# 6dwavenminer/Unsynchronized_Stereo_Vision_Proj325

Measured on NVIDIA B200. Metric: frame-pairs/sec, higher is better.
Workload: dtype u8

## Files before the change

### unsynchronized_stereo_vision_proj325_b200/csrc/usv_capi.cu

```cuda
#include <cuda_runtime.h>

#include <atomic>
#include <cmath>
#include <cstdarg>
#include <cstdio>
#include <algorithm>
#include <cstring>
#include <initializer_list>
#include <memory>
#include <new>
#include <vector>

#include "usv_common.cuh"

namespace usv {
cudaError_t launch_direct(const DevJob& J, int n_pairs, cudaStream_t st);
bool direct_supported(const DevJob& J);
size_t dense_scratch_bytes_per_pair(const DevJob& J);
cudaError_t launch_dense(const DevJob& J, int n_pairs, void* d_scratch, size_t scratch_bytes, cudaStream_t st, const char** kernel_name,
                         int* n_launches);
size_t corr_scratch_bytes_per_pair(const DevJob& J);
cudaError_t launch_dense_corr(const DevJob& J, int n_pairs, void* d_scratch, size_t scratch_bytes, cudaStream_t st, const char** kernel_name,
                              int* n_launches);
cudaError_t launch_contour_descriptors(const int* pts, const int* off, int n, double* desc, cudaStream_t st);
cudaError_t launch_contour_costs(const double* dl, int nl, const double* dr, int nr, double* cost, cudaStream_t st);
size_t resolve_workspace_bytes(long long n);
cudaError_t launch_resolve(const usv_match* d_in, long long n, int skip_unmatched, usv_match* d_out, long long cap, long long* d_n_out,
                           void* d_ws, size_t ws_bytes, cudaStream_t st, int* n_launches);
size_t id_matcher_workspace_bytes(long long n_cur);
bool resolve_rows_supported(int nx, int nxc);
struct ResolveRowsSrc {
  const uint16_t* disparity_u16;
  const uint16_t* raw_cost_u16;
  const uint32_t* raw_cost;
  const uint32_t* right_index;
  const usv_match* matches;
};
cudaError_t launch_resolve_rows(const ResolveRowsSrc& S, bool integer_values, int nx, int ny, int sx, int nxc, long long n_templates,
                                int camera_side, int n_pairs, uint16_t* d_out, cudaStream_t st);
cudaError_t launch_id_matcher(const usv_match* d_cur, long long n_cur, const usv_match* d_old, long long n_old, int* d_out3,
                              long long cap, long long* d_n_out, void* d_ws, size_t ws_bytes, cudaStream_t st);
size_t preprocess_scratch_bytes(int width, int height, int n_frames);
cudaError_t launch_preprocess(int device, const uint8_t* d_src, uint8_t* d_dst, const short* d_map1, const uint16_t* d_map2, int n_frames,
                              int width, int height, int src_stride, int dst_stride, long long src_frame_stride,
                              long long dst_frame_stride, int flavour, int lighting, void* d_scratch, cudaStream_t st, int* n_launches);
cudaError_t run_issue_probe(int which, int sms, double target_ms, double* lane_inst_per_s, uint32_t* d_scratch, cudaStream_t st);
cudaError_t launch_disparity_to_distance(const int* d_disp, long long n, int kind, double* d_out, cudaStream_t st);
cudaError_t launch_build_distance_lut(double* d_lut, int n, int kind, cudaStream_t st);
cudaError_t launch_match_list_distance(const usv_match* d_list, const long long* d_n, long long cap, int nx, int sx, int nxc, int camera_side,
                                       int kind, const double* lut, int lut_n, double* d_out, cudaStream_t st);
cudaError_t launch_moving_object_distance(int camera_side, long long t_this, const float* this_xy, int n_this, const float* other_xy,
                                          int n_other, const float* old_xy, int n_old, const float* older_xy, int n_older,
                                          const int* idx3, int n_idx, long long t_other, long long t_old, long long t_older,
                                          double* out, cudaStream_t st);
cudaError_t launch_coordinate_position(int camera_side, const double* dist, const float* xy, long long n, double* xyz, cudaStream_t st);
cudaError_t launch_subpixel_refine(const DevJob& J, int n_pairs, const uint32_t* d_right_index, int* d_x16, double* d_dist,
                                   cudaStream_t st);
}

namespace usv { int g_sm_count = 148; }

using usv::DevJob;

template <bool kPinned>
struct Buf {
  void* p = nullptr;
  size_t cap = 0;
  Buf() = default;
  Buf(const Buf&) = delete;
  Buf& operator=(const Buf&) = delete;
  Buf(Buf&& o) noexcept : p(o.p), cap(o.cap) { o.p = nullptr; o.cap = 0; }
  ~Buf() { release(); }
  cudaError_t release() {
    const cudaError_t e = !p ? cudaSuccess : kPinned ? cudaFreeHost(p) : cudaFree(p);
    p = nullptr;
    cap = 0;
    return e;
  }
  cudaError_t alloc(size_t bytes, unsigned host_flags = cudaHostAllocDefault) {
    const cudaError_t e = kPinned ? cudaHostAlloc(&p, bytes, host_flags) : cudaMalloc(&p, bytes);
    if (e == cudaSuccess) cap = bytes;
    else p = nullptr;
    return e;
  }
};
using DevBuf = Buf<false>;
using PinnedBuf = Buf<true>;

static const int kNumOut = 9;
static const size_t kOutElem[kNumOut] = {sizeof(usv_match), 4, 4, 8, 8, 4, 2, 2, 2};

struct usv_ctx {
  int device = 0;
  cudaStream_t stream = nullptr;
  char err[512] = {0};
  std::atomic<long long> launches{0};
  const char* last_kernel = "none";
  DevBuf lut[3];
  int lut_n[3] = {0, 0, 0};
  std::vector<DevBuf> retired;
  PinnedBuf status;
  int* d_status = nullptr;
  int corr_kernel = USV_CORR_KERNEL_AUTO;
  std::atomic<int> open_streams{0};
  PinnedBuf pin[3];
  DevBuf in_l, in_r, tx, ty, rows_u32, rows_f64, out[kNumOut], misc[8], resolve_ws, pre_ws, corr_ws, win_ws;
  DevBuf sub_ri, sub_x16, sub_dist;
  ~usv_ctx() { if (stream) cudaStreamDestroy(stream); }
};

static int fail(usv_ctx* c, int code, const char* fmt, ...) {
  if (c) {
    va_list ap;
    va_start(ap, fmt);
    vsnprintf(c->err, sizeof(c->err), fmt, ap);
    va_end(ap);
  }
  return code;
}
#define CU(call)                                                                                         \
  do {                                                                                                   \
    cudaError_t e_ = (call);                                                                             \
    if (e_ != cudaSuccess) return fail(ctx, USV_ERR_CUDA, "%s: %s (%s:%d)", #call, cudaGetErrorString(e_), __FILE__, __LINE__); \
  } while (0)

template <bool kPinned>
static int grow(usv_ctx* ctx, Buf<kPinned>& b, size_t bytes) {
  if (bytes <= b.cap) return USV_OK;
  CU(b.release());
  const size_t want = bytes + bytes / 4 + (kPinned ? 4096 : 256);
  const cudaError_t e = b.alloc(want);
  if (e != cudaSuccess)
    return fail(ctx, USV_ERR_NOMEM, "%s(%zu): %s", kPinned ? "cudaHostAlloc" : "cudaMalloc", want, cudaGetErrorString(e));
  return USV_OK;
}

static const size_t kPairScratchCap = (size_t)3 << 29;

static int grow_pair_scratch(usv_ctx* ctx, DevBuf& ws, size_t per_pair, int32_t n_pairs) {
  size_t want = per_pair * (size_t)n_pairs;
  if (want > kPairScratchCap) want = std::max(per_pair, kPairScratchCap / per_pair * per_pair);
  return grow(ctx, ws, want);
}

struct ArrayOrScratch {
  void** arr;
  size_t bytes;
};
static int or_scratch(usv_ctx* ctx, DevBuf& ws, std::initializer_list<ArrayOrScratch> arrs) {
  size_t total = 0;
  for (const ArrayOrScratch& a : arrs) total += *a.arr ? 0 : a.bytes;
  const int rc = grow(ctx, ws, total);
  if (rc) return rc;
  uint8_t* q = (uint8_t*)ws.p;
  for (const ArrayOrScratch& a : arrs)
    if (!*a.arr) { *a.arr = q; q += a.bytes; }
  return USV_OK;
}

static usv_frame_desc device_frame_desc(const usv_frame_desc* f) {
  usv_frame_desc d = *f;
  d.row_stride = (f->width * f->channels + 127) & ~127;
  d.frame_stride = (int64_t)d.row_stride * f->height;
  return d;
}

static int copy_frames(usv_ctx* ctx, uint8_t* dst, const usv_frame_desc& df, const uint8_t* src, const usv_frame_desc* hf, int32_t n,
                       cudaStream_t st) {
  const int row_bytes = hf->width * hf->channels;
  const bool packed = n == 1 || hf->frame_stride == (int64_t)hf->row_stride * hf->height;
  if (packed && hf->row_stride == df.row_stride) {
    CU(cudaMemcpyAsync(dst, src, (size_t)df.frame_stride * n, cudaMemcpyHostToDevice, st));
  } else if (packed) {
    CU(cudaMemcpy2DAsync(dst, df.row_stride, src, hf->row_stride, row_bytes, (size_t)hf->height * n, cudaMemcpyHostToDevice, st));
  } else {
    for (int i = 0; i < n; ++i)
      CU(cudaMemcpy2DAsync(dst + (size_t)i * df.frame_stride, df.row_stride, src + (size_t)i * hf->frame_stride, hf->row_stride,
                           row_bytes, hf->height, cudaMemcpyHostToDevice, st));
  }
  return USV_OK;
}

static void** out_slot(usv_outputs* o, int i) {
  switch (i) {
    case 0: return (void**)&o->matches;
    case 1: return (void**)&o->right_index;
    case 2: return (void**)&o->raw_cost;
    case 3: return (void**)&o->score;
    case 4: return (void**)&o->distance;
    case 5: return (void**)&o->distance_f32;
    case 6: return (void**)&o->disparity_u16;
    case 7: return (void**)&o->raw_cost_u16;
    default: return (void**)&o->resolved_disparity_u16;
  }
}

static int check_common(usv_ctx* ctx, const usv_frame_desc* f, const usv_search_params* p, int32_t n_pairs) {
  if (!ctx) return USV_ERR_INVALID_ARG;
  if (!f || !p) return fail(ctx, USV_ERR_INVALID_ARG, "null frame/params");
  if (n_pairs < 0 || n_pairs > 65535) return fail(ctx, USV_ERR_INVALID_ARG, "n_pairs %d out of [0, 65535]", n_pairs);
  if (f->width <= 0 || f->height <= 0 || f->channels < 1 || f->channels > 4)
    return fail(ctx, USV_ERR_INVALID_ARG, "bad frame %dx%dx%d", f->width, f->height, f->channels);
  if (f->row_stride < f->width * f->channels) return fail(ctx, USV_ERR_INVALID_ARG, "row_stride %d < width*channels", f->row_stride);
  if (n_pairs > 1 && f->frame_stride < (int64_t)f->row_stride * f->height)
    return fail(ctx, USV_ERR_INVALID_ARG, "frame_stride smaller than one frame");
  if (p->tmpl_w <= 0 || p->tmpl_h <= 0 || p->tmpl_w > f->width || p->tmpl_h > f->height)
    return fail(ctx, USV_ERR_INVALID_ARG, "template %dx%d does not fit frame %dx%d", p->tmpl_w, p->tmpl_h, f->width, f->height);
  if ((int64_t)p->tmpl_w * p->tmpl_h * f->channels > 32768)
    return fail(ctx, USV_ERR_UNSUPPORTED, "template of %lld bytes exceeds 32768 (u32 cost accumulators)",
                (long long)p->tmpl_w * p->tmpl_h * f->channels);
  if (p->tmpl_w * f->channels > 1024) return fail(ctx, USV_ERR_UNSUPPORTED, "template row wider than 1024 bytes");
  if (p->stride_x <= 0 || p->stride_y <= 0) return fail(ctx, USV_ERR_INVALID_ARG, "stride must be positive");
  if (p->search_min > p->search_max) return fail(ctx, USV_ERR_INVALID_ARG, "search_min > search_max");
  if (p->search_min < -(1 << 24) || p->search_max > (1 << 24)) return fail(ctx, USV_ERR_INVALID_ARG, "search range beyond +-2^24");
  if (p->cost_kind < USV_COST_SAD || p->cost_kind > USV_COST_ZNCC) return fail(ctx, USV_ERR_INVALID_ARG, "unknown cost_kind %d", p->cost_kind);
  if (p->distance_kind < USV_DIST_NONE || p->distance_kind > USV_DIST_POWERLAW)
    return fail(ctx, USV_ERR_INVALID_ARG, "unknown distance_kind %d", p->distance_kind);
  if (p->camera_side != USV_LEFT_CAM && p->camera_side != USV_RIGHT_CAM) return fail(ctx, USV_ERR_INVALID_ARG, "camera_side must be 0 or 1");
  return USV_OK;
}

static int check_cost_u16(usv_ctx* ctx, const usv_frame_desc* f, const usv_search_params* p) {
  if (p->cost_kind != USV_COST_SAD || 255ll * p->tmpl_w * p->tmpl_h * f->channels >= 0xFFFFll)
    return fail(ctx, USV_ERR_UNSUPPORTED, "raw_cost_u16 needs SAD with 255*tmpl_w*tmpl_h*channels < 65535");
  return USV_OK;
}

static int check_direct(usv_ctx* ctx, const DevJob& J) {
  if (!usv::direct_supported(J))
    return fail(ctx, USV_ERR_UNSUPPORTED, "template %dx%dx%d: no kernel serves this shape (direct form: shared memory)", J.tw, J.th,
                J.channels);
  return USV_OK;
}

static int check_dev_status(usv_ctx* ctx) {
  volatile int* h_status = (volatile int*)ctx->status.p;
  if (h_status && *h_status != 0) {
    const int s = *h_status;
    *h_status = 0;
    return fail(ctx, USV_ERR_CUDA, "device status %d: a kernel abandoned a wait (results of the affected call are invalid)", s);
  }
  return USV_OK;
}

static void fill_job(usv_ctx* ctx, DevJob& J, const uint8_t* l, const uint8_t* r, const usv_frame_desc* f, const usv_search_params* p,
                     const usv_outputs* o) {
  memset(&J, 0, sizeof(J));
  J.status = ctx->d_status;
  J.corr_kernel = ctx->corr_kernel;
  J.left = l; J.right = r;
  J.frame_stride = f->frame_stride;
  J.width = f->width; J.height = f->height; J.channels = f->channels; J.row_stride = f->row_stride;
  J.tw = p->tmpl_w; J.th = p->tmpl_h; J.dmin = p->search_min; J.dmax = p->search_max;
  J.sx = p->stride_x; J.sy = p->stride_y;
  J.cost_kind = p->cost_kind; J.camera_side = p->camera_side; J.distance_kind = p->distance_kind;
  J.nxc = f->width - p->tmpl_w + 1; J.nyc = f->height - p->tmpl_h + 1;
  J.nx = (J.nxc - 1) / p->stride_x + 1; J.ny = (J.nyc - 1) / p->stride_y + 1;
  J.row_bytes = p->tmpl_w * f->channels;
  J.n_elems = p->tmpl_w * p->tmpl_h * f->channels;
  J.accept_threshold = p->accept_threshold;
  J.n_templates = J.nx * J.ny;
  if (o) J.out = *o;
}

static int ensure_lut(usv_ctx* ctx, int kind, int width, cudaStream_t st, const double** lut) {
  *lut = nullptr;
  if (kind == USV_DIST_NONE) return USV_OK;
  if (ctx->lut_n[kind] < width) {
    if (ctx->lut[kind].p) { ctx->retired.push_back(std::move(ctx->lut[kind])); ctx->lut_n[kind] = 0; }
    int n = width < 4096 ? 4096 : width;
    CU(ctx->lut[kind].alloc(sizeof(double) * n));
    CU(usv::launch_build_distance_lut((double*)ctx->lut[kind].p, n, kind, st));
    CU(cudaStreamSynchronize(st));
    ctx->launches++;
    ctx->lut_n[kind] = n;
  }
  *lut = (const double*)ctx->lut[kind].p;
  return USV_OK;
}

static bool aligned16(const void* p) { return (reinterpret_cast<uintptr_t>(p) & 15) == 0; }

extern "C" int usv_abi_version(void) { return USV_ABI_VERSION; }

extern "C" int usv_create(int device, usv_ctx** out) {
  if (!out) return USV_ERR_INVALID_ARG;
  *out = nullptr;
  int n = 0;
  cudaError_t e = cudaGetDeviceCount(&n);
  if (e != cudaSuccess || n <= 0) return USV_ERR_NO_DEVICE;
  if (device < 0 || device >= n) return USV_ERR_INVALID_ARG;
  if (cudaSetDevice(device) != cudaSuccess) return USV_ERR_CUDA;
  cudaDeviceProp prop;
  if (cudaGetDeviceProperties(&prop, device) != cudaSuccess) return USV_ERR_CUDA;
  if (prop.major != 10 || prop.minor != 0) return USV_ERR_NO_DEVICE;
  usv_ctx* c = new (std::nothrow) usv_ctx();
  if (!c) return USV_ERR_NOMEM;
  c->device = device;
  usv::g_sm_count = prop.multiProcessorCount;
  if (cudaStreamCreateWithFlags(&c->stream, cudaStreamNonBlocking) != cudaSuccess ||
      c->status.alloc(sizeof(int), cudaHostAllocMapped) != cudaSuccess ||
      cudaHostGetDevicePointer((void**)&c->d_status, c->status.p, 0) != cudaSuccess) {
    delete c;
    return USV_ERR_CUDA;
  }
  *(int*)c->status.p = 0;
  *out = c;
  return USV_OK;
}

extern "C" int usv_destroy(usv_ctx* ctx) {
  if (!ctx) return USV_ERR_INVALID_ARG;
  if (ctx->open_streams.load() > 0)
    return fail(ctx, USV_ERR_INVALID_ARG, "%d usv_stream(s) of this context are still open: destroy them first", ctx->open_streams.load());
  cudaSetDevice(ctx->device);
  cudaStreamSynchronize(ctx->stream);
  delete ctx;
  return USV_OK;
}

extern "C" const char* usv_last_error(const usv_ctx* ctx) { return ctx ? ctx->err : "null context"; }
extern "C" int64_t usv_launch_count(const usv_ctx* ctx) { return ctx ? (int64_t)ctx->launches.load() : -1; }
extern "C" const char* usv_last_kernel(const usv_ctx* ctx) { return ctx ? ctx->last_kernel : "none"; }
extern "C" int usv_set_option(usv_ctx* ctx, int32_t key, int64_t value) {
  if (!ctx) return USV_ERR_INVALID_ARG;
  if (key == USV_OPT_CORR_KERNEL) {
    if (value < USV_CORR_KERNEL_AUTO || value > USV_CORR_KERNEL_TCGEN05) return fail(ctx, USV_ERR_INVALID_ARG, "USV_OPT_CORR_KERNEL: value %lld", (long long)value);
    ctx->corr_kernel = (int)value;
    return USV_OK;
  }
  return fail(ctx, USV_ERR_INVALID_ARG, "unknown option %d", key);
}
extern "C" int usv_device_status(usv_ctx* ctx) { return ctx ? check_dev_status(ctx) : USV_ERR_INVALID_ARG; }

extern "C" int usv_grid_dims(const usv_frame_desc* f, const usv_search_params* p, int32_t* nx, int32_t* ny, int64_t* cand_evals) {
  if (!f || !p) return USV_ERR_INVALID_ARG;
  int nxc = f->width - p->tmpl_w + 1, nyc = f->height - p->tmpl_h + 1;
  if (nxc <= 0 || nyc <= 0 || p->stride_x <= 0 || p->stride_y <= 0) return USV_ERR_INVALID_ARG;
  int gx = (nxc - 1) / p->stride_x + 1, gy = (nyc - 1) / p->stride_y + 1;
  int64_t per_row = 0;
  for (int ix = 0; ix < gx; ++ix) {
    int lo, hi;
    usv::cand_range(ix * p->stride_x, nxc, p->camera_side, p->search_min, p->search_max, &lo, &hi);
    if (hi >= lo) per_row += hi - lo + 1;
  }
  if (nx) *nx = gx;
  if (ny) *ny = gy;
  if (cand_evals) *cand_evals = per_row * gy;
  return USV_OK;
}

static int resolve_device(usv_ctx* ctx, const usv_match* d_in, int64_t n, int32_t skip_unmatched, usv_match* d_out, int64_t cap,
                          int64_t* d_n_out, cudaStream_t st);

static int dispatch_match(usv_ctx* ctx, const DevJob& J, int32_t n_pairs, bool sparse, cudaStream_t st, DevBuf* corr_ws) {
  int rc;
  if (!sparse) {
    const char* name = nullptr;
    int nl = 0;
    DevBuf& ws = corr_ws ? *corr_ws : ctx->corr_ws;
    const bool sad_sweep = J.cost_kind == USV_COST_SAD && J.corr_kernel != USV_CORR_KERNEL_ALU;
    if ((rc = grow_pair_scratch(ctx, ws, sad_sweep ? usv::dense_scratch_bytes_per_pair(J) : 0, n_pairs))) return rc;
    cudaError_t e = (J.cost_kind == USV_COST_SAD && J.channels == 3 && J.corr_kernel == USV_CORR_KERNEL_ALU)
                        ? cudaErrorNotSupported
                        : usv::launch_dense(J, n_pairs, ws.p, ws.cap, st, &name, &nl);
    if (e == cudaSuccess) {
      ctx->launches += nl;
      ctx->last_kernel = name;
      return USV_OK;
    }
    if (e != cudaErrorNotSupported) return fail(ctx, USV_ERR_CUDA, "dense launch: %s", cudaGetErrorString(e));
    (void)cudaGetLastError();
    if ((rc = grow_pair_scratch(ctx, ws, usv::corr_scratch_bytes_per_pair(J), n_pairs))) return rc;
    e = usv::launch_dense_corr(J, n_pairs, ws.p, ws.cap, st, &name, &nl);
    if (e == cudaSuccess) {
      ctx->launches += nl;
      ctx->last_kernel = name;
      return USV_OK;
    }
    if (e != cudaErrorNotSupported) return fail(ctx, USV_ERR_CUDA, "dense correlation launch: %s", cudaGetErrorString(e));
    (void)cudaGetLastError();
  }
  if ((rc = check_direct(ctx, J))) return rc;
  cudaError_t e = usv::launch_direct(J, n_pairs, st);
  if (e != cudaSuccess) return fail(ctx, USV_ERR_CUDA, "direct launch: %s", cudaGetErrorString(e));
  ctx->launches++;
  ctx->last_kernel = "block_cost_argmin_direct";
  return USV_OK;
}

enum WinnerSrc { kWinDisparity, kWinRightIndex, kWinMatches };

static WinnerSrc winner_src(const usv_search_params* p, const usv_outputs& o) {
  if (p->cost_kind > USV_COST_SSD) return kWinMatches;
  const bool disp_ok = p->search_min >= 0;
  if (disp_ok && o.disparity_u16 && (o.raw_cost_u16 || o.raw_cost)) return kWinDisparity;
  if (o.right_index && o.raw_cost) return kWinRightIndex;
  return disp_ok ? kWinDisparity : kWinRightIndex;
}

static int match_device(usv_ctx* ctx, const uint8_t* d_left, const uint8_t* d_right, const usv_frame_desc* f, int32_t n_pairs,
                        const usv_search_params* p, const usv_outputs* d_out, const int32_t* d_tx, const int32_t* d_ty,
                        int32_t n_templates, uint32_t* d_cost_rows, double* d_score_rows, int32_t row_cap, cudaStream_t st, DevBuf* corr_ws = nullptr,
                        DevBuf* win_ws = nullptr) {
  int rc = check_common(ctx, f, p, n_pairs);
  if (rc) return rc;
  if (!d_left || !d_right || !d_out) return fail(ctx, USV_ERR_INVALID_ARG, "null device pointer");
  if (!aligned16(d_left) || !aligned16(d_right) || (f->row_stride & 15) || (f->frame_stride & 15))
    return fail(ctx, USV_ERR_INVALID_ARG, "device frames need 16-byte aligned base, row_stride and frame_stride");
  if (d_out->raw_cost_u16 && (rc = check_cost_u16(ctx, f, p))) return rc;
  if (n_pairs == 0) return USV_OK;
  CU(cudaSetDevice(ctx->device));
  DevJob J;
  fill_job(ctx, J, d_left, d_right, f, p, d_out);
  const bool sparse = d_tx != nullptr;
  if (sparse) {
    if (!d_ty || n_templates < 0) return fail(ctx, USV_ERR_INVALID_ARG, "bad template list");
    if (n_templates == 0) return USV_OK;
    J.tx = d_tx; J.ty = d_ty; J.n_templates = n_templates;
    J.cost_rows = d_cost_rows; J.score_rows = d_score_rows; J.row_cap = row_cap;
    if ((d_cost_rows || d_score_rows) && row_cap <= 0) return fail(ctx, USV_ERR_INVALID_ARG, "row_cap must be positive");
  }
  if (J.out.distance || J.out.distance_f32) {
    rc = ensure_lut(ctx, p->distance_kind, f->width, st, &J.dist_lut);
    if (rc) return rc;
  }
  const bool want_resolved = d_out->resolved_disparity_u16 != nullptr;
  const WinnerSrc src = winner_src(p, J.out);
  if (want_resolved) {
    if (sparse) return fail(ctx, USV_ERR_UNSUPPORTED, "resolved_disparity_u16 is an output of the dense sweep");
    if (!usv::resolve_rows_supported(J.nx, J.nxc)) return fail(ctx, USV_ERR_UNSUPPORTED, "resolved_disparity_u16: rows wider than 2048 windows");
    const size_t n_res = (size_t)J.n_templates * n_pairs;
    DevBuf& ws = win_ws ? *win_ws : ctx->win_ws;
    usv_outputs& o = J.out;
    if (src == kWinDisparity)
      rc = or_scratch(ctx, ws, {{o.raw_cost_u16 ? (void**)&o.raw_cost_u16 : (void**)&o.raw_cost, 4 * n_res},
                                {(void**)&o.disparity_u16, 2 * n_res}});
    else if (src == kWinRightIndex)
      rc = or_scratch(ctx, ws, {{(void**)&o.raw_cost, 4 * n_res}, {(void**)&o.right_index, 4 * n_res}});
    else
      rc = or_scratch(ctx, ws, {{(void**)&o.matches, sizeof(usv_match) * n_res}});
    if (rc) return rc;
  }
  if ((rc = dispatch_match(ctx, J, n_pairs, sparse, st, corr_ws))) return rc;
  if (want_resolved) {
    usv::ResolveRowsSrc S;
    memset(&S, 0, sizeof(S));
    if (src == kWinDisparity) {
      S.disparity_u16 = J.out.disparity_u16; S.raw_cost_u16 = J.out.raw_cost_u16; S.raw_cost = J.out.raw_cost;
    } else if (src == kWinRightIndex) {
      S.right_index = J.out.right_index; S.raw_cost = J.out.raw_cost;
    } else {
      S.matches = J.out.matches;
    }
    cudaError_t e = usv::launch_resolve_rows(S, src != kWinMatches, J.nx, J.ny, J.sx, J.nxc, J.n_templates, J.camera_side, n_pairs,
                                             d_out->resolved_disparity_u16, st);
    if (e != cudaSuccess) return fail(ctx, USV_ERR_CUDA, "resolve rows launch: %s", cudaGetErrorString(e));
    ctx->launches++;
  }
  return USV_OK;
}

extern "C" int usv_match_dense_device(usv_ctx* ctx, const uint8_t* d_left, const uint8_t* d_right, const usv_frame_desc* frame,
                                      int32_t n_pairs, const usv_search_params* params, const usv_outputs* d_out, void* cuda_stream) {
  if (!ctx) return USV_ERR_INVALID_ARG;
  return match_device(ctx, d_left, d_right, frame, n_pairs, params, d_out, nullptr, nullptr, 0, nullptr, nullptr, 0,
                      (cudaStream_t)cuda_stream);
}

extern "C" int usv_match_templates_device(usv_ctx* ctx, const uint8_t* d_left, const uint8_t* d_right, const usv_frame_desc* frame,
                                          int32_t n_pairs, const int32_t* d_tx, const int32_t* d_ty, int32_t n_templates,
                                          const usv_search_params* params, const usv_outputs* d_out, uint32_t* d_cost_rows,
                                          double* d_score_rows, int32_t row_cap, void* cuda_stream) {
  if (!ctx) return USV_ERR_INVALID_ARG;
  if (!d_tx) return fail(ctx, USV_ERR_INVALID_ARG, "null template list");
  return match_device(ctx, d_left, d_right, frame, n_pairs, params, d_out, d_tx, d_ty, n_templates, d_cost_rows, d_score_rows,
                      row_cap, (cudaStream_t)cuda_stream);
}

static int check_subpixel(usv_ctx* ctx, const usv_frame_desc* f, const void* x16, const void* dist) {
  if (!x16 && !dist) return fail(ctx, USV_ERR_INVALID_ARG, "sub-pixel refinement: both output pointers are NULL");
  if (f->width > (1 << 26)) return fail(ctx, USV_ERR_UNSUPPORTED, "sub-pixel refinement: frame wider than 2^26 pixels");
  return USV_OK;
}

static int refine_device(usv_ctx* ctx, const uint8_t* d_left, const uint8_t* d_right, const usv_frame_desc* f, int32_t n_pairs,
                         const usv_search_params* p, const uint32_t* d_ri, int32_t* d_x16, double* d_dist, cudaStream_t st) {
  int rc = check_common(ctx, f, p, n_pairs);
  if (rc || (rc = check_subpixel(ctx, f, d_x16, d_dist))) return rc;
  if (!d_left || !d_right || !d_ri) return fail(ctx, USV_ERR_INVALID_ARG, "null device pointer");
  if (!aligned16(d_left) || !aligned16(d_right) || (f->row_stride & 15) || (f->frame_stride & 15))
    return fail(ctx, USV_ERR_INVALID_ARG, "device frames need 16-byte aligned base, row_stride and frame_stride");
  if (n_pairs == 0) return USV_OK;
  CU(cudaSetDevice(ctx->device));
  DevJob J;
  fill_job(ctx, J, d_left, d_right, f, p, nullptr);
  cudaError_t e = usv::launch_subpixel_refine(J, n_pairs, d_ri, d_x16, d_dist, st);
  if (e != cudaSuccess) return fail(ctx, USV_ERR_CUDA, "sub-pixel launch: %s", cudaGetErrorString(e));
  ctx->launches++;
  return USV_OK;
}

extern "C" int usv_refine_subpixel_device(usv_ctx* ctx, const uint8_t* d_left, const uint8_t* d_right, const usv_frame_desc* frame,
                                          int32_t n_pairs, const usv_search_params* params, const uint32_t* d_right_index,
                                          int32_t* d_disparity_x16, double* d_distance, void* cuda_stream) {
  if (!ctx) return USV_ERR_INVALID_ARG;
  return refine_device(ctx, d_left, d_right, frame, n_pairs, params, d_right_index, d_disparity_x16, d_distance,
                       (cudaStream_t)cuda_stream);
}

struct SubpixelOut {
  int32_t* disparity_x16;
  double* distance;
};

static int match_host(usv_ctx* ctx, const uint8_t* h_left, const uint8_t* h_right, const usv_frame_desc* f, int32_t n_pairs,
                      const usv_search_params* p, const usv_outputs* h_out, const int32_t* h_tx, const int32_t* h_ty,
                      int32_t n_templates, uint32_t* h_cost_rows, double* h_score_rows, int32_t row_cap,
                      const SubpixelOut* sub = nullptr) {
  int rc = check_common(ctx, f, p, n_pairs);
  if (rc) return rc;
  if (!h_left || !h_right || !h_out) return fail(ctx, USV_ERR_INVALID_ARG, "null host pointer");
  if (sub && (rc = check_subpixel(ctx, f, sub->disparity_x16, sub->distance))) return rc;
  if (n_pairs == 0) return USV_OK;
  CU(cudaSetDevice(ctx->device));
  cudaStream_t st = ctx->stream;
  const bool sparse = h_tx != nullptr;
  int64_t n_win;
  if (sparse) {
    if (!h_ty || n_templates < 0) return fail(ctx, USV_ERR_INVALID_ARG, "bad template list");
    const int nxc = f->width - p->tmpl_w + 1, nyc = f->height - p->tmpl_h + 1;
    for (int i = 0; i < n_templates; ++i)
      if (h_tx[i] < 0 || h_tx[i] >= nxc || h_ty[i] < 0 || h_ty[i] >= nyc)
        return fail(ctx, USV_ERR_INVALID_ARG, "template %d at (%d,%d) outside the frame", i, h_tx[i], h_ty[i]);
    n_win = n_templates;
    if (n_templates == 0) return USV_OK;
    DevJob J;
    fill_job(ctx, J, nullptr, nullptr, f, p, nullptr);
    if ((rc = check_direct(ctx, J))) return rc;
  } else {
    int32_t nx, ny;
    if (usv_grid_dims(f, p, &nx, &ny, nullptr)) return fail(ctx, USV_ERR_INVALID_ARG, "bad geometry");
    n_win = (int64_t)nx * ny;
  }
  const int64_t n_res = n_win * n_pairs;
  const usv_frame_desc df = device_frame_desc(f);
  const size_t fbytes = (size_t)df.frame_stride * n_pairs;
  if ((rc = grow(ctx, ctx->in_l, fbytes)) || (rc = copy_frames(ctx, (uint8_t*)ctx->in_l.p, df, h_left, f, n_pairs, st))) return rc;
  if ((rc = grow(ctx, ctx->in_r, fbytes)) || (rc = copy_frames(ctx, (uint8_t*)ctx->in_r.p, df, h_right, f, n_pairs, st))) return rc;
  usv_outputs d_out;
  memset(&d_out, 0, sizeof(d_out));
  usv_outputs ho = *h_out;
  for (int i = 0; i < kNumOut; ++i) {
    if (*out_slot(&ho, i)) {
      if ((rc = grow(ctx, ctx->out[i], kOutElem[i] * n_res))) return rc;
      *out_slot(&d_out, i) = ctx->out[i].p;
    }
  }
  int32_t *d_tx = nullptr, *d_ty = nullptr;
  uint32_t* d_rows = nullptr;
  double* d_srows = nullptr;
  if (sparse) {
    if ((rc = grow(ctx, ctx->tx, sizeof(int32_t) * n_templates))) return rc;
    if ((rc = grow(ctx, ctx->ty, sizeof(int32_t) * n_templates))) return rc;
    d_tx = (int32_t*)ctx->tx.p; d_ty = (int32_t*)ctx->ty.p;
    CU(cudaMemcpyAsync(d_tx, h_tx, sizeof(int32_t) * n_templates, cudaMemcpyHostToDevice, st));
    CU(cudaMemcpyAsync(d_ty, h_ty, sizeof(int32_t) * n_templates, cudaMemcpyHostToDevice, st));
    if (h_cost_rows) {
      if ((rc = grow(ctx, ctx->rows_u32, sizeof(uint32_t) * n_res * row_cap))) return rc;
      d_rows = (uint32_t*)ctx->rows_u32.p;
      CU(cudaMemcpyAsync(d_rows, h_cost_rows, sizeof(uint32_t) * n_res * row_cap, cudaMemcpyHostToDevice, st));
    }
    if (h_score_rows) {
      if ((rc = grow(ctx, ctx->rows_f64, sizeof(double) * n_res * row_cap))) return rc;
      d_srows = (double*)ctx->rows_f64.p;
      CU(cudaMemcpyAsync(d_srows, h_score_rows, sizeof(double) * n_res * row_cap, cudaMemcpyHostToDevice, st));
    }
  }
  if (sub && (rc = or_scratch(ctx, ctx->sub_ri, {{(void**)&d_out.right_index, 4 * (size_t)n_res}}))) return rc;
  rc = match_device(ctx, (const uint8_t*)ctx->in_l.p, (const uint8_t*)ctx->in_r.p, &df, n_pairs, p, &d_out, d_tx, d_ty, n_templates,
                    d_rows, d_srows, row_cap, st);
  if (rc) return rc;
  if (sub) {
    int32_t* d_x16 = nullptr;
    double* d_dist = nullptr;
    if (sub->disparity_x16) {
      if ((rc = grow(ctx, ctx->sub_x16, 4 * n_res))) return rc;
      d_x16 = (int32_t*)ctx->sub_x16.p;
    }
    if (sub->distance) {
      if ((rc = grow(ctx, ctx->sub_dist, 8 * n_res))) return rc;
      d_dist = (double*)ctx->sub_dist.p;
    }
    if ((rc = refine_device(ctx, (const uint8_t*)ctx->in_l.p, (const uint8_t*)ctx->in_r.p, &df, n_pairs, p, d_out.right_index, d_x16,
                            d_dist, st)))
      return rc;
    if (d_x16) CU(cudaMemcpyAsync(sub->disparity_x16, d_x16, 4 * n_res, cudaMemcpyDeviceToHost, st));
    if (d_dist) CU(cudaMemcpyAsync(sub->distance, d_dist, 8 * n_res, cudaMemcpyDeviceToHost, st));
  }
  for (int i = 0; i < kNumOut; ++i)
    if (*out_slot(&ho, i)) CU(cudaMemcpyAsync(*out_slot(&ho, i), ctx->out[i].p, kOutElem[i] * n_res, cudaMemcpyDeviceToHost, st));
  if (d_rows) CU(cudaMemcpyAsync(h_cost_rows, d_rows, sizeof(uint32_t) * n_res * row_cap, cudaMemcpyDeviceToHost, st));
  if (d_srows) CU(cudaMemcpyAsync(h_score_rows, d_srows, sizeof(double) * n_res * row_cap, cudaMemcpyDeviceToHost, st));
  CU(cudaStreamSynchronize(st));
  return check_dev_status(ctx);
}

extern "C" int usv_match_dense_host(usv_ctx* ctx, const uint8_t* h_left, const uint8_t* h_right, const usv_frame_desc* frame,
                                    int32_t n_pairs, const usv_search_params* params, const usv_outputs* h_out) {
  if (!ctx) return USV_ERR_INVALID_ARG;
  return match_host(ctx, h_left, h_right, frame, n_pairs, params, h_out, nullptr, nullptr, 0, nullptr, nullptr, 0);
}

extern "C" int usv_match_templates_host(usv_ctx* ctx, const uint8_t* h_left, const uint8_t* h_right, const usv_frame_desc* frame,
                                        int32_t n_pairs, const int32_t* h_tx, const int32_t* h_ty, int32_t n_templates,
                                        const usv_search_params* params, const usv_outputs* h_out, uint32_t* h_cost_rows,
                                        double* h_score_rows, int32_t row_cap) {
  if (!ctx) return USV_ERR_INVALID_ARG;
  if (!h_tx) return fail(ctx, USV_ERR_INVALID_ARG, "null template list");
  return match_host(ctx, h_left, h_right, frame, n_pairs, params, h_out, h_tx, h_ty, n_templates, h_cost_rows, h_score_rows, row_cap);
}

extern "C" int usv_match_dense_subpixel_host(usv_ctx* ctx, const uint8_t* h_left, const uint8_t* h_right, const usv_frame_desc* frame,
                                             int32_t n_pairs, const usv_search_params* params, const usv_outputs* h_out,
                                             int32_t* h_disparity_x16, double* h_distance) {
  if (!ctx) return USV_ERR_INVALID_ARG;
  usv_outputs none;
  memset(&none, 0, sizeof(none));
  const SubpixelOut sub = {h_disparity_x16, h_distance};
  return match_host(ctx, h_left, h_right, frame, n_pairs, params, h_out ? h_out : &none, nullptr, nullptr, 0, nullptr, nullptr, 0, &sub);
}

static int up(usv_ctx* ctx, DevBuf& b, const void* h, size_t bytes) {
  int rc = grow(ctx, b, bytes ? bytes : 16);
  if (rc) return rc;
  if (bytes) CU(cudaMemcpyAsync(b.p, h, bytes, cudaMemcpyHostToDevice, ctx->stream));
  return USV_OK;
}

static int resolve_device(usv_ctx* ctx, const usv_match* d_in, int64_t n, int32_t skip_unmatched, usv_match* d_out, int64_t cap,
                          int64_t* d_n_out, cudaStream_t st) {
  if (n < 0 || cap < 0 || n >= 0x7fffffffll) return fail(ctx, USV_ERR_INVALID_ARG, "match list length %lld out of range", (long long)n);
  if (!d_n_out || (n > 0 && (!d_in || (cap > 0 && !d_out)))) return fail(ctx, USV_ERR_INVALID_ARG, "null pointer");
  CU(cudaSetDevice(ctx->device));
  const size_t ws = n ? usv::resolve_workspace_bytes(n) : 0;
  int rc = grow(ctx, ctx->resolve_ws, ws ? ws : 16);
  if (rc) return rc;
  int nl = 0;
  cudaError_t e = usv::launch_resolve(d_in, n, skip_unmatched, d_out, cap, (long long*)d_n_out, ctx->resolve_ws.p, ws, st, &nl);
  if (e != cudaSuccess) return fail(ctx, USV_ERR_CUDA, "resolve launch: %s", cudaGetErrorString(e));
  ctx->launches += nl;
  if (nl) ctx->last_kernel = "resolve_next_smaller_kernel";
  return USV_OK;
}

extern "C" int usv_resolve_match_list_device(usv_ctx* ctx, const usv_match* d_in, int64_t n, int32_t skip_unmatched, usv_match* d_out,
                                             int64_t cap, int64_t* d_n_out, void* cuda_stream) {
  if (!ctx) return USV_ERR_INVALID_ARG;
  return resolve_device(ctx, d_in, n, skip_unmatched, d_out, cap, d_n_out, (cudaStream_t)cuda_stream);
}

extern "C" int usv_resolve_match_list(usv_ctx* ctx, const usv_match* h_in, int64_t n, int32_t skip_unmatched, usv_match* h_out,
                                      int64_t cap, int64_t* n_out) {
  if (!ctx) return USV_ERR_INVALID_ARG;
  if (n < 0 || cap < 0 || !n_out || (n > 0 && !h_in) || (cap > 0 && !h_out)) return fail(ctx, USV_ERR_INVALID_ARG, "bad arguments");
  *n_out = 0;
  if (n == 0) return USV_OK;
  CU(cudaSetDevice(ctx->device));
  int rc;
  const int64_t room = cap < n ? cap : n;
  if ((rc = up(ctx, ctx->misc[0], h_in, sizeof(usv_match) * (size_t)n))) return rc;
  if ((rc = grow(ctx, ctx->misc[1], sizeof(usv_match) * (size_t)(room ? room : 1)))) return rc;
  if ((rc = grow(ctx, ctx->misc[2], sizeof(int64_t)))) return rc;
  if ((rc = resolve_device(ctx, (const usv_match*)ctx->misc[0].p, n, skip_unmatched, (usv_match*)ctx->misc[1].p, room,
                           (int64_t*)ctx->misc[2].p, ctx->stream)))
    return rc;
  int64_t total = 0;
  CU(cudaMemcpyAsync(&total, ctx->misc[2].p, sizeof(int64_t), cudaMemcpyDeviceToHost, ctx->stream));
  CU(cudaStreamSynchronize(ctx->stream));
  const int64_t m = total < room ? total : room;
  if (m > 0) CU(cudaMemcpy(h_out, ctx->misc[1].p, sizeof(usv_match) * (size_t)m, cudaMemcpyDeviceToHost));
  *n_out = total;
  return USV_OK;
}

extern "C" int usv_block_search_host(usv_ctx* ctx, const uint8_t* h_left, const uint8_t* h_right, const usv_frame_desc* f,
                                     const usv_search_params* p, usv_match* h_matches, double* h_distance, int64_t cap, int64_t* n_out) {
  if (!ctx) return USV_ERR_INVALID_ARG;
  int rc = check_common(ctx, f, p, 1);
  if (rc) return rc;
  if (!h_left || !h_right || !n_out || cap < 0 || (cap > 0 && !h_matches)) return fail(ctx, USV_ERR_INVALID_ARG, "bad arguments");
  *n_out = 0;
  int32_t nx, ny;
  if (usv_grid_dims(f, p, &nx, &ny, nullptr)) return fail(ctx, USV_ERR_INVALID_ARG, "bad geometry");
  const int64_t n_win = (int64_t)nx * ny;
  CU(cudaSetDevice(ctx->device));
  cudaStream_t st = ctx->stream;
  const usv_frame_desc df = device_frame_desc(f);
  const int row_bytes = f->width * f->channels, pitch = df.row_stride;
  const size_t fbytes = (size_t)df.frame_stride;
  if ((rc = grow(ctx, ctx->pin[0], 2 * fbytes))) return rc;
  uint8_t* stage = (uint8_t*)ctx->pin[0].p;
  for (int k = 0; k < 2; ++k) {
    const uint8_t* src = k ? h_right : h_left;
    uint8_t* dst = stage + k * fbytes;
    if (f->row_stride == pitch) memcpy(dst, src, fbytes);
    else for (int y = 0; y < f->height; ++y) memcpy(dst + (size_t)y * pitch, src + (size_t)y * f->row_stride, row_bytes);
  }
  if ((rc = grow(ctx, ctx->in_l, fbytes)) || (rc = grow(ctx, ctx->in_r, fbytes))) return rc;
  CU(cudaMemcpyAsync(ctx->in_l.p, stage, fbytes, cudaMemcpyHostToDevice, st));
  CU(cudaMemcpyAsync(ctx->in_r.p, stage + fbytes, fbytes, cudaMemcpyHostToDevice, st));
  if ((rc = grow(ctx, ctx->out[0], sizeof(usv_match) * n_win))) return rc;
  usv_outputs d_out;
  memset(&d_out, 0, sizeof(d_out));
  d_out.matches = (usv_match*)ctx->out[0].p;
  if ((rc = match_device(ctx, (const uint8_t*)ctx->in_l.p, (const uint8_t*)ctx->in_r.p, &df, 1, p, &d_out, nullptr, nullptr, 0, nullptr,
                         nullptr, 0, st)))
    return rc;
  const char* match_kernel = ctx->last_kernel;
  if ((rc = grow(ctx, ctx->misc[1], sizeof(usv_match) * n_win)) || (rc = grow(ctx, ctx->misc[2], sizeof(int64_t)))) return rc;
  if ((rc = resolve_device(ctx, d_out.matches, n_win, 1, (usv_match*)ctx->misc[1].p, n_win, (int64_t*)ctx->misc[2].p, st))) return rc;
  const bool want_dist = h_distance != nullptr && p->distance_kind != USV_DIST_NONE;
  if (want_dist) {
    const double* lut = nullptr;
    if ((rc = ensure_lut(ctx, p->distance_kind, f->width, st, &lut))) return rc;
    if ((rc = grow(ctx, ctx->misc[3], sizeof(double) * n_win))) return rc;
    CU(usv::launch_match_list_distance((const usv_match*)ctx->misc[1].p, (const long long*)ctx->misc[2].p, n_win, nx, p->stride_x,
                                       f->width - p->tmpl_w + 1, p->camera_side, p->distance_kind, lut, ctx->lut_n[p->distance_kind],
                                       (double*)ctx->misc[3].p, st));
    ctx->launches++;
  }
  ctx->last_kernel = match_kernel;
  if ((rc = grow(ctx, ctx->pin[1], sizeof(usv_match) * n_win + 64)) || (rc = grow(ctx, ctx->pin[2], sizeof(double) * n_win + 64))) return rc;
  int64_t* h_n = (int64_t*)((uint8_t*)ctx->pin[1].p + sizeof(usv_match) * n_win);
  CU(cudaMemcpyAsync(h_n, ctx->misc[2].p, sizeof(int64_t), cudaMemcpyDeviceToHost, st));
  CU(cudaStreamSynchronize(st));
  const int64_t total = *h_n, m = total < cap ? total : cap;
  if (m > 0) {
    CU(cudaMemcpyAsync(ctx->pin[1].p, ctx->misc[1].p, sizeof(usv_match) * (size_t)m, cudaMemcpyDeviceToHost, st));
    if (want_dist) CU(cudaMemcpyAsync(ctx->pin[2].p, ctx->misc[3].p, sizeof(double) * (size_t)m, cudaMemcpyDeviceToHost, st));
    CU(cudaStreamSynchronize(st));
// ... 485 lines not shown
```

### unsynchronized_stereo_vision_proj325_b200/csrc/usv_resolve_rows.cu

```cuda
#include "usv_common.cuh"

namespace usv {

constexpr int kRRThreads = 256;
constexpr int kRRMax = 2048;

__device__ __forceinline__ unsigned long long f64_ordered(double d) {
  const unsigned long long b = (unsigned long long)__double_as_longlong(d);
  return (b >> 63) ? ~b : (b | 0x8000000000000000ull);
}

struct ResolveRowsSrc {
  const uint16_t* disparity_u16;
  const uint16_t* raw_cost_u16;
  const uint32_t* raw_cost;
  const uint32_t* right_index;
  const usv_match* matches;
};

template <typename V>
__global__ void __launch_bounds__(kRRThreads) dense_resolve_rows_kernel(const ResolveRowsSrc S, int nx, int sx, int nxc, long long n_templates,
                                                                         int camera_side, uint16_t* __restrict__ out) {
  extern __shared__ __align__(16) unsigned char rr_smem[];
  V* s_v = reinterpret_cast<V*>(rr_smem);
  V* s_min = s_v + nx;
  int* s_last = reinterpret_cast<int*>(s_min + nxc);
  uint16_t* s_xr = reinterpret_cast<uint16_t*>(s_last + nxc);
  const int iy = blockIdx.x, pair = blockIdx.y, tid = threadIdx.x;
  const long long g0 = (long long)pair * n_templates + (long long)iy * nx;
  const bool left = camera_side == USV_LEFT_CAM;
  for (int k = tid; k < nxc; k += kRRThreads) { s_last[k] = -1; s_min[k] = ~(V)0; }
  for (int i = tid; i < nx; i += kRRThreads) {
    uint32_t xr = 0xFFFFu;
    V v = 0;
    if (sizeof(V) == 4 && S.disparity_u16) {
      const uint32_t d = S.disparity_u16[g0 + i];
      if (d != USV_NO_DISPARITY) {
        xr = (uint32_t)(left ? i * sx - (int)d : i * sx + (int)d);
        v = (V)(S.raw_cost_u16 ? (uint32_t)S.raw_cost_u16[g0 + i] : S.raw_cost[g0 + i]);
      }
    } else if (sizeof(V) == 4 && S.right_index) {
      const uint32_t ri = S.right_index[g0 + i];
      if (ri != USV_NO_MATCH) { xr = ri % (uint32_t)nxc; v = (V)S.raw_cost[g0 + i]; }
    } else {
      const usv_match m = S.matches[g0 + i];
      if (m.RightIndex != USV_NO_MATCH) { xr = m.RightIndex % (uint32_t)nxc; v = (V)f64_ordered(m.MatchValue); }
    }
    s_xr[i] = (uint16_t)xr;
    s_v[i] = v;
  }
  __syncthreads();
  for (int i = tid; i < nx; i += kRRThreads) {
    const uint32_t xr = s_xr[i];
    if (xr != 0xFFFFu) { atomicMax(&s_last[xr], i); atomicMin(&s_min[xr], s_v[i]); }
  }
  __syncthreads();
  for (int i = tid; i < nx; i += kRRThreads) {
    const uint32_t xr = s_xr[i];
    uint16_t r = (uint16_t)USV_NO_DISPARITY;
    if (xr != 0xFFFFu) {
      const V v = s_v[i];
      const int last = s_last[xr];
      bool beaten = false;
      if (v > s_min[xr])
        for (int j = i + 1; j <= last && !beaten; ++j) beaten = s_xr[j] == xr && s_v[j] < v;
      if (!beaten) r = (uint16_t)(left ? i * sx - (int)xr : (int)xr - i * sx);
    }
    out[g0 + i] = r;
  }
}

bool resolve_rows_supported(int nx, int nxc) { return nx <= kRRMax && nxc <= kRRMax; }

cudaError_t launch_resolve_rows(const ResolveRowsSrc& S, bool integer_values, int nx, int ny, int sx, int nxc, long long n_templates,
                                int camera_side, int n_pairs, uint16_t* d_out, cudaStream_t st) {
  if (!resolve_rows_supported(nx, nxc)) return cudaErrorNotSupported;
  const dim3 grid(ny, n_pairs), block(kRRThreads);
  const size_t smem = (size_t)(nx + nxc) * (integer_values ? 4 : 8) + (size_t)nxc * 4 + (size_t)nx * 2 + 16;
  if (integer_values) dense_resolve_rows_kernel<uint32_t><<<grid, block, smem, st>>>(S, nx, sx, nxc, n_templates, camera_side, d_out);
  else dense_resolve_rows_kernel<unsigned long long><<<grid, block, smem, st>>>(S, nx, sx, nxc, n_templates, camera_side, d_out);
  return cudaGetLastError();
}

}
```

Measured before the change: 24990.

## Resolve rows per warp with right-to-left sweep and prefetched segments

Replaces the block-per-row resolve kernel, which used shared atomics and a quadratic forward scan, with a persistent grid in which each warp resolves one row at a time. The warp sweeps right to left, keeping a running per-column minimum and using match_any plus shuffles for collisions inside a 32-wide chunk. It also prefetches the next segment into registers and specializes the loader per source type. Separately, the winner scratch now stores the cost as u16 when SAD is lossless, halving that intermediate traffic. The cost is considerably more complex warp-level logic, where a subtle tie-handling error could change results.

```diff
diff --git a/unsynchronized_stereo_vision_proj325_b200/csrc/usv_capi.cu b/unsynchronized_stereo_vision_proj325_b200/csrc/usv_capi.cu
--- a/unsynchronized_stereo_vision_proj325_b200/csrc/usv_capi.cu
+++ b/unsynchronized_stereo_vision_proj325_b200/csrc/usv_capi.cu
@@ -220,9 +220,12 @@
   return USV_OK;
 }
 
+static bool cost_u16_lossless(const usv_frame_desc* f, const usv_search_params* p) {
+  return p->cost_kind == USV_COST_SAD && 255ll * p->tmpl_w * p->tmpl_h * f->channels < 0xFFFFll;
+}
+
 static int check_cost_u16(usv_ctx* ctx, const usv_frame_desc* f, const usv_search_params* p) {
-  if (p->cost_kind != USV_COST_SAD || 255ll * p->tmpl_w * p->tmpl_h * f->channels >= 0xFFFFll)
-    return fail(ctx, USV_ERR_UNSUPPORTED, "raw_cost_u16 needs SAD with 255*tmpl_w*tmpl_h*channels < 65535");
+  if (!cost_u16_lossless(f, p)) return fail(ctx, USV_ERR_UNSUPPORTED, "raw_cost_u16 needs SAD with 255*tmpl_w*tmpl_h*channels < 65535");
   return USV_OK;
 }
 
@@ -433,10 +436,11 @@
     const size_t n_res = (size_t)J.n_templates * n_pairs;
     DevBuf& ws = win_ws ? *win_ws : ctx->win_ws;
     usv_outputs& o = J.out;
-    if (src == kWinDisparity)
-      rc = or_scratch(ctx, ws, {{o.raw_cost_u16 ? (void**)&o.raw_cost_u16 : (void**)&o.raw_cost, 4 * n_res},
+    if (src == kWinDisparity) {
+      const bool u16 = o.raw_cost_u16 || (!o.raw_cost && cost_u16_lossless(f, p));
+      rc = or_scratch(ctx, ws, {{u16 ? (void**)&o.raw_cost_u16 : (void**)&o.raw_cost, (u16 ? 2 : 4) * n_res},
                                 {(void**)&o.disparity_u16, 2 * n_res}});
-    else if (src == kWinRightIndex)
+    } else if (src == kWinRightIndex)
       rc = or_scratch(ctx, ws, {{(void**)&o.raw_cost, 4 * n_res}, {(void**)&o.right_index, 4 * n_res}});
     else
       rc = or_scratch(ctx, ws, {{(void**)&o.matches, sizeof(usv_match) * n_res}});
diff --git a/unsynchronized_stereo_vision_proj325_b200/csrc/usv_resolve_rows.cu b/unsynchronized_stereo_vision_proj325_b200/csrc/usv_resolve_rows.cu
--- a/unsynchronized_stereo_vision_proj325_b200/csrc/usv_resolve_rows.cu
+++ b/unsynchronized_stereo_vision_proj325_b200/csrc/usv_resolve_rows.cu
@@ -1,9 +1,13 @@
+#include <algorithm>
+
 #include "usv_common.cuh"
 
 namespace usv {
 
-constexpr int kRRThreads = 256;
 constexpr int kRRMax = 2048;
+constexpr int kRRBatch = 8;
+constexpr int kRRSeg = 32 * kRRBatch;
+constexpr uint32_t kRRUnmatched = 0xFFFFu;
 
 __device__ __forceinline__ unsigned long long f64_ordered(double d) {
   const unsigned long long b = (unsigned long long)__double_as_longlong(d);
@@ -18,68 +22,172 @@
   const usv_match* matches;
 };
 
+constexpr int kRRWarps = 4;
 template <typename V>
-__global__ void __launch_bounds__(kRRThreads) dense_resolve_rows_kernel(const ResolveRowsSrc S, int nx, int sx, int nxc, long long n_templates,
-                                                                         int camera_side, uint16_t* __restrict__ out) {
+constexpr int rr_min_ctas() { return sizeof(V) == 4 ? 8 : 6; }
+
+__host__ __device__ constexpr size_t rr_align16(size_t b) { return (b + 15) & ~(size_t)15; }
+
+template <typename V>
+__host__ __device__ size_t rr_warp_bytes(int nxc) {
+  return rr_align16((size_t)nxc * sizeof(V)) + rr_align16((size_t)nxc) + kRRSeg * (sizeof(V) + 2);
+}
+
+enum RRSource { kRRDispCostU16, kRRDispCost, kRRRightIndex, kRRMatches };
+
+template <RRSource kSrc, typename V>
+__device__ __forceinline__ void rr_load(const ResolveRowsSrc& S, long long g0, int base, int lane, int nx, uint32_t (&a)[kRRBatch],
+                                        V (&b)[kRRBatch]) {
+#pragma unroll
+  for (int k = 0; k < kRRBatch; ++k) {
+    const int i = base + lane + 32 * k;
+    const long long g = g0 + i;
+    a[k] = 0;
+    b[k] = 0;
+    if (i >= nx) continue;
+    if constexpr (kSrc == kRRMatches) {
+      a[k] = S.matches[g].RightIndex;
+      b[k] = (V)f64_ordered(S.matches[g].MatchValue);
+    } else {
+      a[k] = kSrc == kRRRightIndex ? S.right_index[g] : S.disparity_u16[g];
+      b[k] = kSrc == kRRDispCostU16 ? (V)S.raw_cost_u16[g] : (V)S.raw_cost[g];
+    }
+  }
+}
+
+template <RRSource kSrc, typename V>
+__device__ __forceinline__ void rr_stage(const uint32_t (&a)[kRRBatch], const V (&b)[kRRBatch], int base, int lane, int nx, int sx,
+                                         int nxc, bool left, uint16_t* s_xr, V* s_v) {
+#pragma unroll
+  for (int k = 0; k < kRRBatch; ++k) {
+    const int i = base + lane + 32 * k;
+    if (i >= nx) continue;
+    uint32_t xr;
+    if constexpr (kSrc == kRRDispCostU16 || kSrc == kRRDispCost)
+      xr = a[k] == USV_NO_DISPARITY ? kRRUnmatched : (uint16_t)(left ? i * sx - (int)a[k] : i * sx + (int)a[k]);
+    else
+      xr = a[k] == USV_NO_MATCH ? kRRUnmatched : (uint16_t)(a[k] % (uint32_t)nxc);
+    s_xr[lane + 32 * k] = (uint16_t)xr;
+    s_v[lane + 32 * k] = b[k];
+  }
+}
+
+template <RRSource kSrc, typename V>
+__device__ __forceinline__ void rr_rows(const ResolveRowsSrc& S, int nx, int ny, int sx, int nxc, long long n_templates, int n_pairs,
+                                        bool left, long long first, int n_warps, int lane, unsigned char* ws, uint16_t* __restrict__ out) {
+  V* const s_min = reinterpret_cast<V*>(ws);
+  uint8_t* const s_tag = ws + rr_align16((size_t)nxc * sizeof(V));
+  V* const s_v = reinterpret_cast<V*>(s_tag + rr_align16((size_t)nxc));
+  uint16_t* const s_xr = reinterpret_cast<uint16_t*>(s_v + kRRSeg);
+  const V kNone = ~(V)0;
+  const unsigned lanes_before = (1u << lane) - 1, lanes_after = 0xFFFFFFFEu << lane;
+  uint4* const min16 = reinterpret_cast<uint4*>(s_min);
+  const int n_min16 = (int)(rr_align16((size_t)nxc * sizeof(V)) / 16);
+  const uint4 none16 = make_uint4(~0u, ~0u, ~0u, ~0u);
+  for (int k = lane; k < n_min16; k += 32) min16[k] = none16;
+
+  const int last_seg = (nx - 1) / kRRSeg * kRRSeg;
+  long long pair = first / ny;
+  int iy = (int)(first % ny);
+  uint32_t a[kRRBatch];
+  V b[kRRBatch];
+  if (pair < n_pairs) rr_load<kSrc>(S, pair * n_templates + (long long)iy * nx, last_seg, lane, nx, a, b);
+  while (pair < n_pairs) {
+    const long long g0 = pair * n_templates + (long long)iy * nx;
+    int next_iy = iy + n_warps;
+    const long long next_pair = pair + next_iy / ny;
+    next_iy %= ny;
+    uint16_t* const orow = out + g0;
+    for (int base = last_seg; base >= 0; base -= kRRSeg) {
+      rr_stage<kSrc>(a, b, base, lane, nx, sx, nxc, left, s_xr, s_v);
+      __syncwarp();
+      if (base > 0)
+        rr_load<kSrc>(S, g0, base - kRRSeg, lane, nx, a, b);
+      else if (next_pair < n_pairs)
+        rr_load<kSrc>(S, next_pair * n_templates + (long long)next_iy * nx, last_seg, lane, nx, a, b);
+      for (int c0 = min(base + kRRSeg, (nx + 31) & ~31) - 32; c0 >= base; c0 -= 32) {
+        const int i = c0 + lane;
+        const bool in = i < nx;
+        const uint32_t xr = in ? s_xr[i - base] : kRRUnmatched;
+        const V v = in ? s_v[i - base] : kNone;
+        const bool matched = xr != kRRUnmatched;
+        if (matched) s_tag[xr] = (uint8_t)lane;
+        __syncwarp();
+        unsigned same = 1u << lane;
+        V group_min = v;
+        V after = kNone;
+        if (__any_sync(~0u, matched && s_tag[xr] != lane)) {
+          same = __match_any_sync(~0u, matched ? xr : 0x10000u + lane);
+          const unsigned later = same & lanes_after;
+          const int next = later ? __ffs(later) - 1 : lane;
+          const int rounds = 32 - __clz(__reduce_max_sync(~0u, __popc(same)) - 1);
+          int p = next;
+          for (int r = 0; r < rounds; ++r) {
+            const V m = __shfl_sync(~0u, group_min, p);
+            p = __shfl_sync(~0u, p, p);
+            group_min = m < group_min ? m : group_min;
+          }
+          const V m = __shfl_sync(~0u, group_min, next);
+          if (later) after = m;
+        }
+        const V seen = matched ? s_min[xr] : kNone;
+        __syncwarp();
+        if (matched && !(same & lanes_before) && group_min < seen) s_min[xr] = group_min;
+        const int d = left ? i * sx - (int)xr : (int)xr - i * sx;
+        if (in) orow[i] = matched && v <= seen && v <= after ? (uint16_t)d : (uint16_t)USV_NO_DISPARITY;
+      }
+      __syncwarp();
+    }
+    for (int k = lane; k < n_min16; k += 32) min16[k] = none16;
+    __syncwarp();
+    pair = next_pair;
+    iy = next_iy;
+  }
+}
+
+template <typename V>
+__global__ void __launch_bounds__(32 * kRRWarps, rr_min_ctas<V>()) dense_resolve_rows_kernel(const ResolveRowsSrc S, int nx, int ny, int sx, int nxc,
+                                                                                         long long n_templates, int n_pairs, int camera_side,
+                                                                                         uint16_t* __restrict__ out) {
   extern __shared__ __align__(16) unsigned char rr_smem[];
-  V* s_v = reinterpret_cast<V*>(rr_smem);
-  V* s_min = s_v + nx;
-  int* s_last = reinterpret_cast<int*>(s_min + nxc);
-  uint16_t* s_xr = reinterpret_cast<uint16_t*>(s_last + nxc);
-  const int iy = blockIdx.x, pair = blockIdx.y, tid = threadIdx.x;
-  const long long g0 = (long long)pair * n_templates + (long long)iy * nx;
+  const int lane = threadIdx.x & 31, warp = threadIdx.x >> 5;
+  unsigned char* const ws = rr_smem + (size_t)warp * rr_warp_bytes<V>(nxc);
   const bool left = camera_side == USV_LEFT_CAM;
-  for (int k = tid; k < nxc; k += kRRThreads) { s_last[k] = -1; s_min[k] = ~(V)0; }
-  for (int i = tid; i < nx; i += kRRThreads) {
-    uint32_t xr = 0xFFFFu;
-    V v = 0;
-    if (sizeof(V) == 4 && S.disparity_u16) {
-      const uint32_t d = S.disparity_u16[g0 + i];
-      if (d != USV_NO_DISPARITY) {
-        xr = (uint32_t)(left ? i * sx - (int)d : i * sx + (int)d);
-        v = (V)(S.raw_cost_u16 ? (uint32_t)S.raw_cost_u16[g0 + i] : S.raw_cost[g0 + i]);
-      }
-    } else if (sizeof(V) == 4 && S.right_index) {
-      const uint32_t ri = S.right_index[g0 + i];
-      if (ri != USV_NO_MATCH) { xr = ri % (uint32_t)nxc; v = (V)S.raw_cost[g0 + i]; }
-    } else {
-      const usv_match m = S.matches[g0 + i];
-      if (m.RightIndex != USV_NO_MATCH) { xr = m.RightIndex % (uint32_t)nxc; v = (V)f64_ordered(m.MatchValue); }
-    }
-    s_xr[i] = (uint16_t)xr;
-    s_v[i] = v;
-  }
-  __syncthreads();
-  for (int i = tid; i < nx; i += kRRThreads) {
-    const uint32_t xr = s_xr[i];
-    if (xr != 0xFFFFu) { atomicMax(&s_last[xr], i); atomicMin(&s_min[xr], s_v[i]); }
-  }
-  __syncthreads();
-  for (int i = tid; i < nx; i += kRRThreads) {
-    const uint32_t xr = s_xr[i];
-    uint16_t r = (uint16_t)USV_NO_DISPARITY;
-    if (xr != 0xFFFFu) {
-      const V v = s_v[i];
-      const int last = s_last[xr];
-      bool beaten = false;
-      if (v > s_min[xr])
-        for (int j = i + 1; j <= last && !beaten; ++j) beaten = s_xr[j] == xr && s_v[j] < v;
-      if (!beaten) r = (uint16_t)(left ? i * sx - (int)xr : (int)xr - i * sx);
-    }
-    out[g0 + i] = r;
-  }
+  const long long first = (long long)blockIdx.x * kRRWarps + warp;
+  const int n_warps = gridDim.x * kRRWarps;
+  if constexpr (sizeof(V) == 8)
+    rr_rows<kRRMatches, V>(S, nx, ny, sx, nxc, n_templates, n_pairs, left, first, n_warps, lane, ws, out);
+  else if (S.disparity_u16 && S.raw_cost_u16)
+    rr_rows<kRRDispCostU16, V>(S, nx, ny, sx, nxc, n_templates, n_pairs, left, first, n_warps, lane, ws, out);
+  else if (S.disparity_u16)
+    rr_rows<kRRDispCost, V>(S, nx, ny, sx, nxc, n_templates, n_pairs, left, first, n_warps, lane, ws, out);
+  else
+    rr_rows<kRRRightIndex, V>(S, nx, ny, sx, nxc, n_templates, n_pairs, left, first, n_warps, lane, ws, out);
 }
 
 bool resolve_rows_supported(int nx, int nxc) { return nx <= kRRMax && nxc <= kRRMax; }
 
+template <typename V>
+static cudaError_t launch_rr(const ResolveRowsSrc& S, int nx, int ny, int sx, int nxc, long long n_templates, int camera_side, int n_pairs,
+                             uint16_t* d_out, cudaStream_t st) {
+  const auto k = dense_resolve_rows_kernel<V>;
+  const int threads = 32 * kRRWarps;
+  const size_t smem = kRRWarps * rr_warp_bytes<V>(nxc);
+  cudaError_t e = cudaFuncSetAttribute(k, cudaFuncAttributeMaxDynamicSharedMemorySize, (int)smem);
+  if (e != cudaSuccess) return e;
+  int ctas_per_sm = 0;
+  if ((e = cudaOccupancyMaxActiveBlocksPerMultiprocessor(&ctas_per_sm, k, threads, smem)) != cudaSuccess) return e;
+  const long long rows = (long long)ny * n_pairs;
+  const long long ctas = std::min((rows + kRRWarps - 1) / kRRWarps, (long long)std::max(ctas_per_sm, 1) * g_sm_count);
+  k<<<(unsigned)ctas, threads, smem, st>>>(S, nx, ny, sx, nxc, n_templates, n_pairs, camera_side, d_out);
+  return cudaGetLastError();
+}
+
 cudaError_t launch_resolve_rows(const ResolveRowsSrc& S, bool integer_values, int nx, int ny, int sx, int nxc, long long n_templates,
                                 int camera_side, int n_pairs, uint16_t* d_out, cudaStream_t st) {
   if (!resolve_rows_supported(nx, nxc)) return cudaErrorNotSupported;
-  const dim3 grid(ny, n_pairs), block(kRRThreads);
-  const size_t smem = (size_t)(nx + nxc) * (integer_values ? 4 : 8) + (size_t)nxc * 4 + (size_t)nx * 2 + 16;
-  if (integer_values) dense_resolve_rows_kernel<uint32_t><<<grid, block, smem, st>>>(S, nx, sx, nxc, n_templates, camera_side, d_out);
-  else dense_resolve_rows_kernel<unsigned long long><<<grid, block, smem, st>>>(S, nx, sx, nxc, n_templates, camera_side, d_out);
-  return cudaGetLastError();
+  return integer_values ? launch_rr<uint32_t>(S, nx, ny, sx, nxc, n_templates, camera_side, n_pairs, d_out, st)
+                        : launch_rr<unsigned long long>(S, nx, ny, sx, nxc, n_templates, camera_side, n_pairs, d_out, st);
 }
 
 }
```

Result: faster. 25580, median of 6 (+2.3%).
